# flynn-nrg/izpi

Measured on AMD Instinct MI355X. Metric: Msamples/sec (pixels x spp) at 1024x1024/512spp, higher is better.
Workload: dtype f64

## Files before the change

### izpi_amd/csrc/izpi_dev.h

```cpp
#pragma once
#include <hip/hip_runtime.h>
#include <stdint.h>
#include "../../include/izpi_gpu.h"
#include "gomath.h"

#define IZPI_DEV __device__ __forceinline__

namespace izd {

__host__ __device__ inline bool ref_is_leaf(int32_t r) { return r <= -2; }
__host__ __device__ inline int32_t leaf_start(int32_t r) { return (-r - 1) >> 3; }
__host__ __device__ inline int32_t leaf_count(int32_t r) { return (-r - 1) & 7; }
__host__ __device__ inline int32_t make_leaf_ref(int32_t start, int32_t count) { return -(1 + ((start << 3) | count)); }

struct alignas(16) GInner {
  float mnx[4], mny[4], mnz[4], mxx[4], mxy[4], mxz[4];
  int32_t child[4];
  int32_t pad[4];
};
struct alignas(64) GInnerQ {
  float org[3];
  uint32_t ex;
  uint32_t q[6];
  int32_t child[4];
  uint32_t pad[2];
};
static_assert(sizeof(GInnerQ) == 64, "GInnerQ is 64 B");
__host__ __device__ inline float qdecode(float org, uint32_t q, float s) {
  const float p = (float)q * s;
  return org + p;
}
struct alignas(16) GLeaf {
  float mn[3], mx[3];
  int32_t start, count;
};
struct alignas(16) GPrim {
  double a[9];
  uint32_t kind;
  uint32_t index;
};
struct alignas(32) GShade {
  double n[3];
  uint32_t ref;
  uint32_t mk;
};
__host__ __device__ inline uint32_t gs_mat(const GShade& g) { return g.mk >> 8; }
__host__ __device__ inline uint32_t gs_kind(const GShade& g) { return (g.mk >> 2) & 63u; }
__host__ __device__ inline uint32_t gs_cflags(const GShade& g) { return g.mk & 3u; }
struct alignas(16) GTriTex {
  double uv[6];
  double tg[3], bt[3];
};
struct alignas(16) GTriVerts {
  double v1[3], v2[3];
};
struct alignas(16) GLight {
  double v0[3], v1[3], v2[3], e1[3], e2[3], n[3];
  double area;
  double c0[3], c1[3], radius, t0, t1;
  double cz[3];
  uint32_t kind, index;
};

enum { TEXF_RGBA = 0, TEXF_GRAY = 1, TEXF_OTHER = 2, TEXF_NONE = 3 };
struct alignas(16) TexSlot {
  uint64_t off;
  uint32_t w, hf;
};
struct alignas(64) MatTex {
  TexSlot s[4];
};

struct DevScene {
  const GInner* inner;
  const GInnerQ* innerq;
  const GLeaf* leaves;
  const GPrim* prims;
  const GShade* shade;
  const GTriTex* tritex;
  const GLight* lights;
  const izpi_material* materials;
  const izpi_texture* textures;
  const double4* mat_const;
  const MatTex* mat_tex;
  const double* texels;
  const double* spd_wl;
  const double* spd_val;
  int32_t root;
  uint32_t num_lights;
  uint32_t nan_free_bounds;
  uint32_t leaf_shortcut;
  uint32_t tri_only;
  uint32_t no_pathlen;
  uint32_t num_inner;
  uint32_t num_prims;
  izpi_camera cam;
  uint32_t lds_bytes;
  uint32_t time_free;
  uint32_t quantized;
#ifdef IZPI_SHADOW
  const GInner* sh_inner;
  const GLeaf* sh_leaves;
  const GPrim* sh_prims;
#endif
};

struct RenderParams {
  uint32_t width, height, spp, max_depth;
  uint32_t chunk_spp;
  uint32_t s0;
  uint32_t num_pixels;
  uint32_t tile_w, tile_h;
  uint32_t total_units;
  uint32_t lanes;
  uint32_t num_bg_spd;
  const uint32_t* tiles;
  const double* bg_wl;
  const double* bg_val;
  double background[3];
  uint64_t seed;
  double* out;
  double* recs;
  uint32_t* head;
  unsigned long long* counters;
  uint32_t* error;
};

struct Lcg {
  uint32_t s;
  IZPI_DEV double next() {
    s = 1664525u * s + 1013904223u;
    return (double)s / 4294967296.0;
  }
};
IZPI_DEV uint64_t splitmix64(uint64_t x) {
  uint64_t z = x + 0x9E3779B97F4A7C15ull;
  z = (z ^ (z >> 30)) * 0xBF58476D1CE4E5B9ull;
  z = (z ^ (z >> 27)) * 0x94D049BB133111EBull;
  return z ^ (z >> 31);
}
#define IZPI_CAMERA_STREAM_SALT 0xD6E8FEB86659FD93ull

IZPI_DEV int64_t go_int(double x) {
  if (x != x || x >= 9223372036854775808.0 || x < -9223372036854775808.0) return INT64_MIN;
  return (int64_t)x;
}

struct V3 { double x, y, z; };
IZPI_DEV V3 mk(double x, double y, double z) { V3 r; r.x = x; r.y = y; r.z = z; return r; }
IZPI_DEV V3 ld3(const double* p) { return mk(p[0], p[1], p[2]); }
IZPI_DEV V3 add(V3 a, V3 b) { return mk(a.x + b.x, a.y + b.y, a.z + b.z); }
IZPI_DEV V3 sub(V3 a, V3 b) { return mk(a.x - b.x, a.y - b.y, a.z - b.z); }
IZPI_DEV V3 mul(V3 a, V3 b) { return mk(a.x * b.x, a.y * b.y, a.z * b.z); }
IZPI_DEV V3 smul(V3 a, double t) { return mk(a.x * t, a.y * t, a.z * t); }
IZPI_DEV bool sdiv_plain(double x) {
  return ((uint32_t)(__double2hiint(x) >> 20) & 0x7FFu) - (1023u - 300u) <= 600u;
}
IZPI_DEV V3 sdiv(V3 a, double t) {
  const int px = (int)sdiv_plain(a.x) | (int)(a.x == 0.0), py = (int)sdiv_plain(a.y) | (int)(a.y == 0.0),
            pz = (int)sdiv_plain(a.z) | (int)(a.z == 0.0);
  const bool plain = ((int)sdiv_plain(t) & px & py & pz) != 0;
  if (plain) {
    double r = __builtin_amdgcn_rcp(t);
    double e = __builtin_fma(-t, r, 1.0);
    r = __builtin_fma(r, e, r);
    e = __builtin_fma(-t, r, 1.0);
    r = __builtin_fma(r, e, r);
    auto q1 = [&](double n) {
      const double q = n * r;
      const double res = __builtin_fma(-t, q, n);
      return __builtin_amdgcn_div_fixup(__builtin_amdgcn_div_fmas(res, r, q, false), t, n);
    };
    return mk(q1(a.x), q1(a.y), q1(a.z));
  }
  return mk(a.x / t, a.y / t, a.z / t);
}
IZPI_DEV double dot(V3 a, V3 b) { return (a.x * b.x) + (a.y * b.y) + (a.z * b.z); }
IZPI_DEV V3 cross(V3 a, V3 b) { return mk((a.y * b.z) - (a.z * b.y), -((a.x * b.z) - (a.z * b.x)), (a.x * b.y) - (a.y * b.x)); }
IZPI_DEV double sqlen(V3 a) { return (a.x * a.x) + (a.y * a.y) + (a.z * a.z); }
IZPI_DEV double length(V3 a) { return gm::sqrt(sqlen(a)); }
IZPI_DEV V3 unit(V3 a) { return sdiv(a, length(a)); }
IZPI_DEV V3 lerp(V3 a, V3 b, double t) {
  return mk((1 - t) * a.x + t * b.x, (1 - t) * a.y + t * b.y, (1 - t) * a.z + t * b.z);
}
IZPI_DEV bool bad(double x) { return x != x || gm::is_inf(x, 0); }
IZPI_DEV V3 denan(V3 v) { return mk(bad(v.x) ? 0.0 : v.x, bad(v.y) ? 0.0 : v.y, bad(v.z) ? 0.0 : v.z); }

struct Onb {
  V3 u, v, w;
  IZPI_DEV void build(V3 n) {
    w = unit(n);
    V3 a = gm::abs(w.x) > 0.9 ? mk(0, 1, 0) : mk(1, 0, 0);
    v = unit(cross(w, a));
    u = cross(w, v);
  }
  IZPI_DEV V3 local(V3 a) const { return add(add(smul(u, a.x), smul(v, a.y)), smul(w, a.z)); }
};

IZPI_DEV V3 random_cosine_direction(Lcg& r) {
  double r1 = r.next();
  double r2 = r.next();
  double z = gm::sqrt(1 - r2);
  double phi = 6.283185307179586 * r1;
  double sp, cp;
  gm::sincos_nonneg(phi, &sp, &cp);
  double x = cp * 2 * gm::sqrt(r2);
  double y = sp * 2 * gm::sqrt(r2);
  return mk(x, y, z);
}
IZPI_DEV V3 random_to_sphere(double radius, double dist2, Lcg& r) {
  double r1 = r.next();
  double r2 = r.next();
  double z = 1 + r2 * (gm::sqrt(1 - radius * radius / dist2) - 1);
  double phi = 6.283185307179586 * r1;
  double sp, cp;
  gm::sincos_nonneg(phi, &sp, &cp);
  double x = cp * gm::sqrt(1 - z * z);
  double y = sp * gm::sqrt(1 - z * z);
  return mk(x, y, z);
}
IZPI_DEV V3 random_in_unit_sphere(Lcg& r) {
  for (;;) {
    double x = r.next(), y = r.next(), z = r.next();
    V3 p = sub(smul(mk(x, y, z), 2.0), mk(1.0, 1.0, 1.0));
    if (sqlen(p) < 1.0) return p;
  }
}

IZPI_DEV float max32(float a, float b) { return a > b ? a : b; }
IZPI_DEV float min32(float a, float b) { return a < b ? a : b; }
IZPI_DEV bool slab(float mnx, float mny, float mnz, float mxx, float mxy, float mxz, float ox, float oy, float oz,
                   float ix, float iy, float iz, float tmax) {
  float t0x = (mnx - ox) * ix, t1x = (mxx - ox) * ix;
  if (t0x > t1x) { float t = t0x; t0x = t1x; t1x = t; }
  float t0y = (mny - oy) * iy, t1y = (mxy - oy) * iy;
  if (t0y > t1y) { float t = t0y; t0y = t1y; t1y = t; }
  float t0z = (mnz - oz) * iz, t1z = (mxz - oz) * iz;
  if (t0z > t1z) { float t = t0z; t0z = t1z; t1z = t; }
  float tn = max32(max32(t0x, t0y), t0z);
  float tf = min32(min32(t1x, t1y), t1z);
  return tn <= tf && tf >= 0 && tn <= tmax;
}

typedef float f32x2 __attribute__((ext_vector_type(2)));
IZPI_DEV uint32_t slab4_fast(float4 mnx, float4 mny, float4 mnz, float4 mxx, float4 mxy, float4 mxz, float ox, float oy,
                             float oz, float ix, float iy, float iz, float tmax) {
  const f32x2 o_x = {ox, ox}, o_y = {oy, oy}, o_z = {oz, oz};
  const f32x2 i_x = {ix, ix}, i_y = {iy, iy}, i_z = {iz, iz};
  const f32x2 a0x = (f32x2{mnx.x, mnx.y} - o_x) * i_x, a1x = (f32x2{mnx.z, mnx.w} - o_x) * i_x;
  const f32x2 b0x = (f32x2{mxx.x, mxx.y} - o_x) * i_x, b1x = (f32x2{mxx.z, mxx.w} - o_x) * i_x;
  const f32x2 a0y = (f32x2{mny.x, mny.y} - o_y) * i_y, a1y = (f32x2{mny.z, mny.w} - o_y) * i_y;
  const f32x2 b0y = (f32x2{mxy.x, mxy.y} - o_y) * i_y, b1y = (f32x2{mxy.z, mxy.w} - o_y) * i_y;
  const f32x2 a0z = (f32x2{mnz.x, mnz.y} - o_z) * i_z, a1z = (f32x2{mnz.z, mnz.w} - o_z) * i_z;
  const f32x2 b0z = (f32x2{mxz.x, mxz.y} - o_z) * i_z, b1z = (f32x2{mxz.z, mxz.w} - o_z) * i_z;
  const float t0x[4] = {a0x.x, a0x.y, a1x.x, a1x.y}, t1x[4] = {b0x.x, b0x.y, b1x.x, b1x.y};
  const float t0y[4] = {a0y.x, a0y.y, a1y.x, a1y.y}, t1y[4] = {b0y.x, b0y.y, b1y.x, b1y.y};
  const float t0z[4] = {a0z.x, a0z.y, a1z.x, a1z.y}, t1z[4] = {b0z.x, b0z.y, b1z.x, b1z.y};
  uint32_t m = 0;
#pragma unroll
  for (int i = 0; i < 4; i++) {
    const float tn = __builtin_fmaxf(__builtin_fmaxf(__builtin_fminf(t0x[i], t1x[i]), __builtin_fminf(t0y[i], t1y[i])),
                                     __builtin_fminf(t0z[i], t1z[i]));
    const float tf = __builtin_fminf(__builtin_fminf(__builtin_fmaxf(t0x[i], t1x[i]), __builtin_fmaxf(t0y[i], t1y[i])),
                                     __builtin_fmaxf(t0z[i], t1z[i]));
    m |= (tn <= tf && tf >= 0.0f && tn <= tmax) ? (1u << i) : 0u;
  }
  return m;
}
IZPI_DEV bool ray_fast_ok(float ox, float oy, float oz, float ix, float iy, float iz) {
  const float inf = __builtin_huge_valf();
  return __builtin_fabsf(ox) < inf && __builtin_fabsf(oy) < inf && __builtin_fabsf(oz) < inf &&
         __builtin_fabsf(ix) < inf && __builtin_fabsf(iy) < inf && __builtin_fabsf(iz) < inf &&
         ix != 0.0f && iy != 0.0f && iz != 0.0f;
}

IZPI_DEV bool tri_intersect(const double* a, V3 o, V3 d, double tmin, double tmax, double& t, double& u, double& v) {
  const double eps = 1e-8;
  V3 v0 = mk(a[0], a[1], a[2]), e1 = mk(a[3], a[4], a[5]), e2 = mk(a[6], a[7], a[8]);
  V3 h = cross(d, e2);
  double aa = dot(e1, h);
  if (gm::abs(aa) < eps) return false;
  double f = 1.0 / aa;
  V3 s = sub(o, v0);
  u = f * dot(s, h);
  if (u < -eps || u > 1.0 + eps) return false;
  V3 q = cross(s, e1);
  v = f * dot(d, q);
  if (v < -eps || u + v > 1.0 + eps) return false;
  t = f * dot(e2, q);
  if (t < tmin || t > tmax) return false;
  return true;
}
IZPI_DEV bool tri_intersect_no_tmax(const double* a, V3 o, V3 d, double tmin, double& t, double& u, double& v) {
  const double eps = 1e-8;
  V3 v0 = mk(a[0], a[1], a[2]), e1 = mk(a[3], a[4], a[5]), e2 = mk(a[6], a[7], a[8]);
  V3 h = cross(d, e2);
  double aa = dot(e1, h);
  if (gm::abs(aa) < eps) return false;
  double f = 1.0 / aa;
  V3 s = sub(o, v0);
  u = f * dot(s, h);
  if (u < -eps || u > 1.0 + eps) return false;
  V3 q = cross(s, e1);
  v = f * dot(d, q);
  if (v < -eps || u + v > 1.0 + eps) return false;
  t = f * dot(e2, q);
  if (t < tmin) return false;
  return true;
}
IZPI_DEV V3 sph_center(const double* a, double time) {
  V3 c0 = mk(a[0], a[1], a[2]), c1 = mk(a[3], a[4], a[5]);
  return add(c0, smul(sub(c1, c0), ((time - a[7]) / (a[8] - a[7]))));
}
IZPI_DEV bool sph_intersect_at(V3 center, double radius, V3 o, V3 d, double tmin, double tmax, double& t, int& root) {
  V3 oc = sub(o, center);
  double aa = dot(d, d);
  double b = dot(oc, d);
  double c = dot(oc, oc) - (radius * radius);
  double disc = (b * b) - (aa * c);
  if (disc > 0) {
    double temp = (-b - gm::sqrt(b * b - aa * c)) / aa;
    if (temp < tmax && temp > tmin) { t = temp; root = 0; return true; }
    temp = (-b + gm::sqrt(b * b - aa * c)) / aa;
    if (temp < tmax && temp > tmin) { t = temp; root = 1; return true; }
  }
  return false;
}
IZPI_DEV bool sph_roots(V3 center, double radius, V3 o, V3 d, double& t0, double& t1) {
  V3 oc = sub(o, center);
  double aa = dot(d, d);
  double b = dot(oc, d);
  double c = dot(oc, oc) - (radius * radius);
  double disc = (b * b) - (aa * c);
  if (!(disc > 0)) return false;
  t0 = (-b - gm::sqrt(b * b - aa * c)) / aa;
  t1 = (-b + gm::sqrt(b * b - aa * c)) / aa;
  return true;
}
IZPI_DEV bool sph_intersect(const double* a, V3 o, V3 d, double time, double tmin, double tmax, double& t, int& root) {
  return sph_intersect_at(sph_center(a, time), a[6], o, d, tmin, tmax, t, root);
}

}
```

### izpi_amd/csrc/trace.hip

```cpp
#include "izpi_kern.h"

constexpr uint32_t BVH_LDS_BYTES = 4096;
template <int S, int WPE, bool DIST, bool TRI, bool LB, bool RL, bool Q>
__global__ void __launch_bounds__(256) __attribute__((amdgpu_waves_per_eu(WPE))) k_trace2(const DevScene sc, const WaveParams wp, unsigned long long* counters,
                                                uint32_t* err, int32_t* spill, uint32_t spill_stride, uint32_t prim_w,
                                                uint32_t tchunk, uint32_t refill_min) {
  static_assert((S & (S - 1)) == 0, "ring size must be a power of two");
  static_assert(!LB || DIST, "the LDS-resident BVH instance runs the distributed leaf tests");
  static_assert(!RL || (DIST && (TRI || LB)), "the LDS-resident ray instances: triangle-only global BVH, or the BVH in LDS");
  static_assert(!Q || !LB, "the quantised nodes are read from global memory");
  constexpr bool UVL = !RL, UVS = RL && LB, DUV = !RL || LB;
  typedef float v4f __attribute__((ext_vector_type(4)));
  typedef double v2d __attribute__((ext_vector_type(2)));
  typedef const __attribute__((address_space(3))) v4f LF4;
  typedef const __attribute__((address_space(3))) v2d LD2;
  __shared__ float4 bvh_lds[LB ? BVH_LDS_BYTES / 16 : 1];
  LF4* const l_inner = (LF4*)bvh_lds;
  LF4* const l_leaves = l_inner + (size_t)8 * (LB ? sc.num_inner : 0);
  LD2* const l_prims = (LD2*)(l_leaves + (size_t)2 * (LB ? sc.num_prims : 0));
  if constexpr (LB) {
    const uint32_t ni = 8 * sc.num_inner, nl = 2 * sc.num_prims, np5 = 5 * sc.num_prims;
    for (uint32_t t = threadIdx.x; t < ni + nl + np5; t += 256)
      bvh_lds[t] = t < ni ? reinterpret_cast<const float4*>(sc.inner)[t]
                          : (t < ni + nl ? reinterpret_cast<const float4*>(sc.leaves)[t - ni]
                                         : reinterpret_cast<const float4*>(sc.prims)[t - ni - nl]);
    __syncthreads();
  }
  __shared__ int32_t lds_stack[S * 256];
  __shared__ uint32_t dist_owner[DIST ? 260 : 1];
  __shared__ double dist_t[DIST ? 260 : 1], dist_u[DIST && DUV ? 260 : 1], dist_v[DIST && DUV ? 260 : 1];
  __shared__ double2 lds_uv[UVL ? 256 : 1];
  __shared__ double2 ray_lds[RL ? 3 * 256 : 1];
  const uint32_t wbase = threadIdx.x & ~63u;
  int32_t* stk = lds_stack + threadIdx.x;
  int32_t* gsp = spill + blockIdx.x * 256 + threadIdx.x;
  const uint32_t lane = threadIdx.x & 63;
  const uint32_t n = *wp.in_count;
  if (wp.pool_ctr && blockIdx.x == 0) pool_publish(wp.pool_ctr);
  if (wp.out_count && blockIdx.x == 0 && threadIdx.x == 0) *wp.out_count = 0;
  if (wp.out_park && blockIdx.x == 0 && threadIdx.x == 0) *wp.out_park = 0;
  const bool read_kind = wp.read_kind != 0 || (wp.in_park && *wp.in_park != 0);
  const uint32_t nwaves = gridDim.x * 4u;
  const uint32_t chunk = min(tchunk, max(16u, (n + nwaves - 1u) / nwaves));
  const uint32_t first = chunk;
  if ((uint64_t)(blockIdx.x * 4u + (threadIdx.x >> 6)) * first >= n) return;
  uint64_t c_rays = 0, c_nodes = 0, c_tri = 0, c_sph = 0;
  uint64_t c_nstep = 0, c_pstep = 0, c_short = 0;
  bool busy = false, in_prim = false;
  bool exhausted = false;
  uint32_t qi = 0;
  uint32_t lkind = RAY_MAIN;
  double tmax = 0;
  float ix = 0, iy = 0, iz = 0, ox = 0, oy = 0, oz = 0;
  int32_t cur = -1, pk = 0, pend = 0;
  int sp = 0, low = 0;
  int clean_from = 0;
  int32_t bprim = -1;
  bool fast = false;
#ifdef IZPI_SHADOW
  uint64_t c_spill_st = 0, c_spill_ld = 0;
  uint32_t sh_acc = 0;
#endif
  uint32_t c_pos = __builtin_amdgcn_readfirstlane((blockIdx.x * 4u + (threadIdx.x >> 6)) * first);
  uint32_t c_end = c_pos + first < n ? c_pos + first : n;
#ifdef IZPI_TRACE_CLOCKS
  uint64_t k_refill = 0, k_node = 0, k_prim = 0, k_adv = 0, k0 = 0, k1 = 0;
#define IZPI_CLK(v) (v) = __builtin_readcyclecounter()
#else
#define IZPI_CLK(v) (void)0
#endif
  for (;;) {
    IZPI_CLK(k0);
    const uint64_t idle = __ballot(!busy);
    if (idle != 0) {
      const uint32_t nidle = (uint32_t)__popcll(idle);
      if (!exhausted && (nidle >= refill_min || idle == ~0ull) && c_pos >= c_end) {
        uint32_t b = 0;
        if (lane == 0) b = atomicAdd(wp.trace_next, chunk);
        b = __builtin_amdgcn_readfirstlane(b) + nwaves * first;
        if (b >= n) exhausted = true;
        c_pos = b;
        c_end = b + chunk < n ? b + chunk : n;
      }
      if (!exhausted && (nidle >= refill_min || idle == ~0ull) && c_pos < c_end) {
        const uint32_t take = nidle < c_end - c_pos ? nidle : c_end - c_pos;
        const uint32_t base = c_pos;
        c_pos += take;
        bool main_ray = false;
        const uint32_t rank = (uint32_t)__popcll(idle & ((1ull << lane) - 1));
        const uint32_t my = base + rank;
        if (!busy && rank < take) {
          const uint32_t k = read_kind ? sld(wp.in.kind + my) : (uint32_t)RAY_MAIN;
          RayOD r;
          if constexpr (RL) {
            r = sld(wp.in.ray + my);
            const double2* rp = reinterpret_cast<const double2*>(&r);
            const double2 r0 = rp[0], r1 = rp[1], r2 = rp[2];
            ray_lds[3 * threadIdx.x] = r0; ray_lds[3 * threadIdx.x + 1] = r1; ray_lds[3 * threadIdx.x + 2] = r2;
          } else {
            r = wp.in.ray[my];
          }
          if (!(k & (RAY_PARKED | RAY_DEAD)) && (uint64_t)__double_as_longlong(r.o[0]) != DEAD_BITS) {
            qi = my;
            lkind = k;
            tmax = ray_tmax(wp.in, my, k);
            main_ray = kind_of(k) == RAY_MAIN;
            ix = (float)(1.0 / r.d[0]); iy = (float)(1.0 / r.d[1]); iz = (float)(1.0 / r.d[2]);
            ox = (float)r.o[0]; oy = (float)r.o[1]; oz = (float)r.o[2];
            fast = sc.nan_free_bounds && ray_fast_ok(ox, oy, oz, ix, iy, iz);
            cur = sc.root;
            sp = 0; low = 0; clean_from = 0;
            in_prim = false;
            bprim = -1;
            busy = cur != -1;
            if (!busy) {
              if ((UVL || UVS) && wp.hit_uv) {
                double2* rec = wp.in.hit + ((size_t)my << 1);
                sst(rec, hit_pack(0.0, -1)); sst(rec + 1, make_double2(0.0, 0.0));
              } else {
                sst(wp.in.hit + my, hit_pack(0.0, -1));
              }
            }
          }
        }
        c_rays += (uint64_t)__popcll(__ballot(main_ray));
        __builtin_amdgcn_s_waitcnt(0x0F70);
      } else if (exhausted && idle == ~0ull) {
        break;
      }
    }
    const uint64_t m_prim = __ballot(busy && in_prim);
    const uint64_t m_node = __ballot(busy && !in_prim);
    if ((m_prim | m_node) == 0) continue;
    const uint32_t n_prim = (uint32_t)__popcll(m_prim), n_node = (uint32_t)__popcll(m_node);
    bool advance = false;
    bool leaf_next = false;
    int32_t next = -1;
#ifdef IZPI_TRACE_CLOCKS
    IZPI_CLK(k1); k_refill += k1 - k0; k0 = k1;
    const bool clk_prim = n_prim * prim_w >= n_node * 16u;
#endif
    if (n_prim * prim_w >= n_node * 16u) {
      if constexpr (DIST) {
        const uint32_t cnt = (busy && in_prim) ? (uint32_t)(pend - pk) : 0u;
        const uint64_t lt = (1ull << lane) - 1;
        const uint32_t base = (uint32_t)__popcll(__ballot(cnt & 1u) & lt) + 2u * (uint32_t)__popcll(__ballot(cnt & 2u) & lt) +
                              4u * (uint32_t)__popcll(__ballot(cnt & 4u) & lt);
        const bool served = cnt > 0 && base + cnt <= 64;
        const uint64_t ms = __ballot(served);
        const int last = 63 - __clzll((long long)ms);
        const uint32_t total = (uint32_t)__shfl((int)(base + cnt), last);
        {
          const uint32_t e = ((uint32_t)pk << 6) | lane;
          uint32_t* dq = dist_owner + wbase + base;
          if (served) dq[0] = e;
          if (served && cnt > 1) dq[1] = e + 64u;
          if (served && cnt > 2) dq[2] = e + 128u;
          if (served && cnt > 3) dq[3] = e + 192u;
        }
        __builtin_amdgcn_wave_barrier();
        const uint32_t ent = lane < total ? dist_owner[wbase + lane] : lane;
        const uint32_t ow = ent & 63u;
        const uint32_t oqi = (uint32_t)__shfl((int)qi, (int)ow);
        const uint32_t okind = (uint32_t)__shfl((int)lkind, (int)ow);
        if (lane < total) {
          const int32_t pi = (int32_t)(ent >> 6);
          double2 r0, r1, r2;
          if constexpr (RL) {
            const uint32_t ro = 3 * (wbase + ow);
            r0 = ray_lds[ro]; r1 = ray_lds[ro + 1]; r2 = ray_lds[ro + 2];
          } else {
            const double2* rp = reinterpret_cast<const double2*>(wp.in.ray + oqi);
            r0 = rp[0]; r1 = rp[1]; r2 = rp[2];
          }
          const double otmin = ray_tmin(wp.in, oqi, okind);
          double2 p0, p1, p2, p3, p4;
          if constexpr (LB) {
            LD2* pp = l_prims + (size_t)5 * pi;
            const v2d a0 = pp[0], a1 = pp[1], a2 = pp[2], a3 = pp[3], a4 = pp[4];
            p0 = make_double2(a0.x, a0.y); p1 = make_double2(a1.x, a1.y); p2 = make_double2(a2.x, a2.y);
            p3 = make_double2(a3.x, a3.y); p4 = make_double2(a4.x, a4.y);
          } else {
            const double2* pp = reinterpret_cast<const double2*>(sc.prims + pi);
            p0 = pp[0]; p1 = pp[1]; p2 = pp[2]; p3 = pp[3]; p4 = pp[4];
#ifdef IZPI_SHADOW
            if (IZPI_SHADOW & 4) {
              const uint4* sq = reinterpret_cast<const uint4*>(sc.sh_prims + pi);
              const uint4 s0 = sq[0], s1 = sq[1], s2 = sq[2], s3 = sq[3], s4 = sq[4];
              sh_acc ^= s0.x ^ s1.y ^ s2.z ^ s3.w ^ s4.x;
            }
#endif
          }
          const double pa[9] = {p0.x, p0.y, p1.x, p1.y, p2.x, p2.y, p3.x, p3.y, p4.x};
          double t = 0, u = 0, v = 0;
          const V3 o = mk(r0.x, r0.y, r1.x), d = mk(r1.y, r2.x, r2.y);
          uint32_t flags;
          if (TRI || (uint32_t)__double2loint(p4.y) == IZPI_PRIM_TRIANGLE) {
            flags = tri_intersect_no_tmax(pa, o, d, otmin, t, u, v) ? 1u : 0u;
          } else {
            const double time = (RL && LB) || sc.time_free ? pa[7] : (wp.in.time ? wp.in.time[oqi] : 0.0);
            flags = 2u;
            if (sph_roots(sph_center(pa, time), pa[6], o, d, t, u))
              flags |= 1u | (t > otmin ? 4u : 0u) | (u > otmin ? 8u : 0u);
          }
          dist_t[wbase + lane] = t;
          if constexpr (DUV) { dist_u[wbase + lane] = u; dist_v[wbase + lane] = v; }
          dist_owner[wbase + lane] = flags;
        }
        const uint32_t n_sph_tests = TRI ? 0u : (uint32_t)__popcll(__ballot(lane < total && (dist_owner[wbase + lane] & 2u)));
        __builtin_amdgcn_wave_barrier();
        if (served && (TRI || n_sph_tests == 0)) {
          const uint32_t j0 = wbase + base;
          uint32_t f[4];
          double tt[4];
#pragma unroll
          for (uint32_t i = 0; i < 4; i++) { f[i] = dist_owner[j0 + i]; tt[i] = dist_t[j0 + i]; }
          int32_t acc = -1;
#pragma unroll
          for (uint32_t i = 0; i < 4; i++)
            if (i < cnt && (f[i] & 1u) && !(tt[i] > tmax)) { tmax = tt[i]; acc = (int32_t)i; }
          if (acc >= 0) {
            if constexpr (UVL) lds_uv[threadIdx.x] = make_double2(dist_u[j0 + acc], dist_v[j0 + acc]);
            if constexpr (UVS)
              if (wp.hit_uv) sst(wp.in.hit + ((size_t)qi << 1) + 1, make_double2(dist_u[j0 + acc], dist_v[j0 + acc]));
            bprim = pk + acc;
            clean_from = sp;
          }
          pk = pend;
          in_prim = false;
          advance = true;
        } else if (!TRI && served) {
          int32_t acc = -1;
          double acc_u = 0, acc_v = 0;
          for (uint32_t i = 0; i < cnt; i++) {
            const uint32_t j = wbase + base + i;
            const uint32_t f = dist_owner[j];
            if (!(f & 1u)) continue;
            if (!(f & 2u)) {
              const double t = dist_t[j];
              if (!(t > tmax)) { tmax = t; acc = (int32_t)j; acc_u = dist_u[j]; acc_v = dist_v[j]; bprim = pk + (int32_t)i; }
            } else {
              const double ta = dist_t[j], tb = dist_u[j];
              if (ta < tmax && (f & 4u)) { tmax = ta; acc = (int32_t)j; acc_u = 0.0; acc_v = 0.0; bprim = pk + (int32_t)i; }
              else if (tb < tmax && (f & 8u)) { tmax = tb; acc = (int32_t)j; acc_u = 1.0; acc_v = 0.0; bprim = pk + (int32_t)i; }
            }
          }
          if (acc >= 0) {
            if constexpr (UVS) {
              if (wp.hit_uv) sst(wp.in.hit + ((size_t)qi << 1) + 1, make_double2(acc_u, acc_v));
            } else {
              lds_uv[threadIdx.x] = make_double2(acc_u, acc_v);
            }
            clean_from = sp;
          }
          pk = pend;
          in_prim = false;
          advance = true;
        }
        __builtin_amdgcn_wave_barrier();
        c_tri += total - n_sph_tests;
        c_sph += n_sph_tests;
        c_pstep++;
      } else {
      bool is_tri = false;
      if (busy && in_prim) {
        const double2* rp = reinterpret_cast<const double2*>(wp.in.ray + qi);
        const double2 r0 = rp[0], r1 = rp[1], r2 = rp[2];
        const V3 o = mk(r0.x, r0.y, r1.x), d = mk(r1.y, r2.x, r2.y);
        const double tmin = ray_tmin(wp.in, qi, lkind);
        const double2* pp = reinterpret_cast<const double2*>(sc.prims + pk);
        const double2 p0 = pp[0], p1 = pp[1], p2 = pp[2], p3 = pp[3], p4 = pp[4];
        const double pa[9] = {p0.x, p0.y, p1.x, p1.y, p2.x, p2.y, p3.x, p3.y, p4.x};
        is_tri = TRI || (uint32_t)__double2loint(p4.y) == IZPI_PRIM_TRIANGLE;
        if (is_tri) {
          double t, u, v;
          if (tri_intersect(pa, o, d, tmin, tmax, t, u, v)) {
            tmax = t; bprim = pk; lds_uv[threadIdx.x] = make_double2(u, v); clean_from = sp;
          }
        } else if (!TRI) {
          const double time = wp.in.time ? wp.in.time[qi] : 0.0;
          double t; int root;
          if (sph_intersect(pa, o, d, time, tmin, tmax, t, root)) {
            tmax = t; bprim = pk; lds_uv[threadIdx.x] = make_double2((double)root, 0.0); clean_from = sp;
          }
        }
        pk++;
        if (pk == pend) { in_prim = false; advance = true; }
      }
      const uint32_t n_tri = (uint32_t)__popcll(__ballot(is_tri));
      c_tri += n_tri;
      c_sph += n_prim - n_tri;
      c_pstep++;
      }
    } else {
      c_nodes += n_node;
      c_nstep++;
      const bool wave_fast = __ballot(busy && !in_prim && !fast) == 0;
      if (__ballot(busy && !in_prim && sp + 3 - low > S) != 0) {
        if (busy && !in_prim) {
          while (sp + 3 - low > S) {
            gsp[(size_t)low * spill_stride] = stk[(low & (S - 1)) * 256];
            low++;
#ifdef IZPI_SHADOW
            c_spill_st++;
#endif
          }
        }
      }
      if (busy && !in_prim) {
        const float tm = (float)tmax;
        const bool is_leaf = ref_is_leaf(cur);
        float4 q0, q1, mnz_, mxx_, mxy_, mxz_;
        int4 ch_;
        if constexpr (LB) {
          LF4* lp = is_leaf ? l_leaves + (size_t)2 * leaf_start(cur) : l_inner + (size_t)8 * cur;
          LF4* np = is_leaf ? l_inner : lp;
          const v4f a0 = lp[0], a1 = lp[1], a2 = np[2], a3 = np[3], a4 = np[4], a5 = np[5], c = np[6];
          q0 = make_float4(a0.x, a0.y, a0.z, a0.w); q1 = make_float4(a1.x, a1.y, a1.z, a1.w);
          mnz_ = make_float4(a2.x, a2.y, a2.z, a2.w); mxx_ = make_float4(a3.x, a3.y, a3.z, a3.w);
          mxy_ = make_float4(a4.x, a4.y, a4.z, a4.w); mxz_ = make_float4(a5.x, a5.y, a5.z, a5.w);
          ch_ = make_int4(__float_as_int(c.x), __float_as_int(c.y), __float_as_int(c.z), __float_as_int(c.w));
        } else if constexpr (Q) {
          const float4* lp = reinterpret_cast<const float4*>(is_leaf ? (const void*)(sc.leaves + leaf_start(cur))
                                                                     : (const void*)(sc.innerq + cur));
          const float4* np = is_leaf ? reinterpret_cast<const float4*>(sc.innerq) : lp;
          q0 = lp[0]; q1 = lp[1];
          const float4 c2 = np[2], c3 = np[3];
          const uint32_t ex = __float_as_uint(q0.w);
          const float sx = __uint_as_float((ex & 0xFFu) << 23), sy = __uint_as_float(((ex >> 8) & 0xFFu) << 23),
                      sz = __uint_as_float(((ex >> 16) & 0xFFu) << 23);
          auto dec4 = [](float w, float o, float sc_) {
            const uint32_t b = __float_as_uint(w);
            return make_float4(__builtin_fmaf((float)(b & 0xFFu), sc_, o), __builtin_fmaf((float)((b >> 8) & 0xFFu), sc_, o),
                               __builtin_fmaf((float)((b >> 16) & 0xFFu), sc_, o), __builtin_fmaf((float)(b >> 24), sc_, o));
          };
          const float4 dmnx = dec4(q1.x, q0.x, sx), dmny = dec4(q1.y, q0.y, sy), dmnz = dec4(q1.z, q0.z, sz);
          const float4 dmxx = dec4(q1.w, q0.x, sx), dmxy = dec4(c2.x, q0.y, sy), dmxz = dec4(c2.y, q0.z, sz);
          const float4 l0 = q0, l1 = q1;
          q0 = is_leaf ? l0 : dmnx;
          q1 = is_leaf ? l1 : make_float4(dmny.x, dmny.y, dmny.z, dmny.w);
          mnz_ = dmnz; mxx_ = dmxx; mxy_ = dmxy; mxz_ = dmxz;
          ch_ = make_int4(__float_as_int(c2.z), __float_as_int(c2.w), __float_as_int(c3.x), __float_as_int(c3.y));
        } else {
          const float4* lp = reinterpret_cast<const float4*>(is_leaf ? (const void*)(sc.leaves + leaf_start(cur))
                                                                     : (const void*)(sc.inner + cur));
          const float4* np = is_leaf ? reinterpret_cast<const float4*>(sc.inner) : lp;
          q0 = lp[0]; q1 = lp[1];
          mnz_ = np[2]; mxx_ = np[3]; mxy_ = np[4]; mxz_ = np[5];
          ch_ = *reinterpret_cast<const int4*>(np + 6);
#ifdef IZPI_SHADOW
          if ((IZPI_SHADOW & 1) && !is_leaf) {
            const uint4* sq = reinterpret_cast<const uint4*>(sc.sh_inner + cur);
            const uint4 s0 = sq[0], s1 = sq[1], s2 = sq[2], s3 = sq[3], s4 = sq[4], s5 = sq[5], s6 = sq[6];
            sh_acc ^= s0.x ^ s1.y ^ s2.z ^ s3.w ^ s4.x ^ s5.y ^ s6.z;
          }
          if ((IZPI_SHADOW & 2) && is_leaf) {
            const uint4* sq = reinterpret_cast<const uint4*>(sc.sh_leaves + leaf_start(cur));
            const uint4 s0 = sq[0], s1 = sq[1];
            sh_acc ^= s0.x ^ s1.y;
          }
#endif
        }
        const float4 mnx = q0;
        const float4 mny = make_float4(is_leaf ? q0.y : q1.x, q1.y, q1.z, q1.w);
        const float4 mnz = make_float4(is_leaf ? q0.z : mnz_.x, mnz_.y, mnz_.z, mnz_.w);
        const float4 mxx = make_float4(is_leaf ? q0.w : mxx_.x, mxx_.y, mxx_.z, mxx_.w);
        const float4 mxy = make_float4(is_leaf ? q1.x : mxy_.x, mxy_.y, mxy_.z, mxy_.w);
        const float4 mxz = make_float4(is_leaf ? q1.y : mxz_.x, mxz_.y, mxz_.z, mxz_.w);
        const int4 ch = make_int4(is_leaf ? cur : ch_.x, ch_.y, ch_.z, ch_.w);
        uint32_t hm;
        if (wave_fast) {
          hm = slab4_fast(mnx, mny, mnz, mxx, mxy, mxz, ox, oy, oz, ix, iy, iz, tm);
        } else {
          const float amnx[4] = {mnx.x, mnx.y, mnx.z, mnx.w}, amny[4] = {mny.x, mny.y, mny.z, mny.w},
                      amnz[4] = {mnz.x, mnz.y, mnz.z, mnz.w}, amxx[4] = {mxx.x, mxx.y, mxx.z, mxx.w},
                      amxy[4] = {mxy.x, mxy.y, mxy.z, mxy.w}, amxz[4] = {mxz.x, mxz.y, mxz.z, mxz.w};
          hm = 0;
#pragma unroll
          for (int i = 0; i < 4; i++)
            if (slab(amnx[i], amny[i], amnz[i], amxx[i], amxy[i], amxz[i], ox, oy, oz, ix, iy, iz, tm)) hm |= 1u << i;
        }
        const uint32_t valid = is_leaf ? 1u
                                       : ((ch.x != -1 ? 1u : 0u) | (ch.y != -1 ? 2u : 0u) | (ch.z != -1 ? 4u : 0u) |
                                          (ch.w != -1 ? 8u : 0u));
        const uint32_t m = hm & valid;
        const int32_t c01 = (m & 1u) ? ch.x : ch.y, c23 = (m & 4u) ? ch.z : ch.w;
        next = m == 0 ? -1 : ((m & 3u) ? c01 : c23);
        const bool enter = ref_is_leaf(next) && (is_leaf || sc.leaf_shortcut);
        leaf_next = enter && !is_leaf;
        in_prim = enter;
        pk = enter ? leaf_start(next) : pk;
        pend = enter ? leaf_start(next) + leaf_count(next) : pend;
        next = enter ? -1 : next;
        const uint32_t rest = m & (m - 1u);
        const int np_ = __builtin_popcount(rest);
        const int32_t e0 = (rest & 2u) ? ch.y : ((rest & 4u) ? ch.z : ch.w);
        const int32_t e1 = ((rest & 6u) == 6u) ? ch.z : ch.w;
        stk[(sp & (S - 1)) * 256] = e0;
        stk[((sp + 1) & (S - 1)) * 256] = e1;
        stk[((sp + 2) & (S - 1)) * 256] = ch.w;
        if (sp + np_ > 64) atomicOr(err, 1u);
        sp += np_;
        advance = !enter;
      }
    }
#ifdef IZPI_TRACE_CLOCKS
    IZPI_CLK(k1); if (clk_prim) k_prim += k1 - k0; else k_node += k1 - k0; k0 = k1;
#endif
    {
      const bool do_pop = advance && next == -1 && sp > 0;
      const bool do_fin = advance && next == -1 && sp == 0;
      const int spn = sp - 1;
      int32_t top = *(volatile __attribute__((address_space(3))) int32_t*)&lds_stack[threadIdx.x + (spn & (S - 1)) * 256];
      if (__ballot(do_pop && spn < low) != 0) {
        if (do_pop && spn < low) {
          top = gsp[(size_t)spn * spill_stride];
          low = spn;
#ifdef IZPI_SHADOW
          c_spill_ld++;
#endif
        }
        __builtin_amdgcn_s_waitcnt(0x0F70);
      }
      cur = (advance && next != -1) ? next : (do_pop ? top : cur);
      sp = do_pop ? spn : sp;
      const bool lf = do_pop && ref_is_leaf(top) && spn >= clean_from && sc.leaf_shortcut;
      in_prim = in_prim || lf;
      leaf_next = leaf_next || lf;
      pk = lf ? leaf_start(top) : pk;
      pend = lf ? leaf_start(top) + leaf_count(top) : pend;
      clean_from = (do_pop && spn < clean_from) ? spn : clean_from;
      if (do_fin) {
        const double2 uv = (UVL && bprim >= 0) ? lds_uv[threadIdx.x] : make_double2(0.0, 0.0);
        if ((UVL || UVS) && wp.hit_uv) {
          double2* rec = wp.in.hit + ((size_t)qi << 1);
          sst(rec, hit_pack(bprim >= 0 ? tmax : 0.0, bprim));
          if (!UVS || bprim < 0) sst(rec + 1, uv);
        } else {
          sst(wp.in.hit + qi, hit_pack(bprim >= 0 ? tmax : 0.0, bprim));
        }
        busy = false;
      }
    }
    const uint64_t n_short = (uint64_t)__popcll(__ballot(leaf_next));
    c_nodes += n_short;
    c_short += n_short;
#ifdef IZPI_TRACE_CLOCKS
    IZPI_CLK(k1); k_adv += k1 - k0;
#endif
  }
#ifdef IZPI_TRACE_CLOCKS
  if (lane == 0) {
    atomicAdd(counters + CNT_CLK_REFILL, (unsigned long long)k_refill);
    atomicAdd(counters + CNT_CLK_NODE, (unsigned long long)k_node);
    atomicAdd(counters + CNT_CLK_PRIM, (unsigned long long)k_prim);
    atomicAdd(counters + CNT_CLK_ADV, (unsigned long long)k_adv);
  }
#endif
#ifdef IZPI_SHADOW
  {
    if (c_spill_st) atomicAdd(counters + CNT_CLK_REFILL, (unsigned long long)c_spill_st);
    if (c_spill_ld) atomicAdd(counters + CNT_CLK_NODE, (unsigned long long)c_spill_ld);
    if (sh_acc == 0x9E3779B9u) atomicOr(err, 0u);
  }
#endif
  if (lane == 0) {
    count_add(wp.cpart, counters, CNT_RAYS, c_rays);
    count_add(wp.cpart, counters, CNT_NODES, c_nodes);
    count_add(wp.cpart, counters, CNT_TRI, c_tri);
    count_add(wp.cpart, counters, CNT_SPH, c_sph);
    count_add(wp.cpart, counters, CNT_NSTEP, c_nstep);
    count_add(wp.cpart, counters, CNT_PSTEP, c_pstep);
    count_add(wp.cpart, counters, CNT_SHORT, c_short);
  }
}


#define IZPI_T2_LIST(X)                                                                                           \
  X(true, false, false, false, false) X(true, true, false, false, false) X(false, false, false, false, false)        \
  X(false, true, false, false, false) X(true, false, true, false, false) X(true, true, true, false, false)           \
  X(true, true, false, true, false) X(true, false, true, true, false) X(true, true, true, true, false)               \
  X(true, false, false, false, true) X(true, true, false, false, true) X(true, true, false, true, true)
constexpr int ring_of(bool lb, bool rl) { return lb && rl ? 8 : TRACE_RING; }

int make_tracer(izpi_ctx* ctx, const izpi_render_tuning& tu, bool need_uv, Tracer* t) {
  *t = Tracer();
  if (tu.flags & IZPI_TUNE_NO_DIST) t->p2 = false;
  if (ctx->num_prims >= (1u << 26)) t->p2 = false;
  t->tri = ctx->sc.tri_only != 0 && !(tu.flags & IZPI_TUNE_GENERAL_TRACE);
  t->lds_bvh = t->p2 && !(tu.flags & IZPI_TUNE_NO_LDS_BVH) &&
               (uint64_t)ctx->sc.num_inner * sizeof(GInner) + (uint64_t)ctx->sc.num_prims * (sizeof(GLeaf) + sizeof(GPrim)) <= BVH_LDS_BYTES;
  if (t->lds_bvh) {
    t->refill_min = 40;
    t->prim_w = 24;
  }
  t->ray_lds = t->p2 && ((t->tri && !t->lds_bvh && !need_uv) || (t->lds_bvh && (t->tri || ctx->sc.time_free))) &&
               !(tu.flags & IZPI_TUNE_NO_RAY_LDS);
  t->qnodes = ctx->sc.quantized && t->p2 && !t->lds_bvh && !(tu.flags & IZPI_TUNE_NO_QNODES);
  if (tu.prim_weight) t->prim_w = tu.prim_weight;
  if (tu.trace_chunk) t->tchunk = tu.trace_chunk;
  if (tu.refill_min) t->refill_min = std::min<uint32_t>(64, tu.refill_min);
  int rc = IZPI_ERR_INVALID;
  ctx->err = "no k_trace2 instance for this scene and tuning";
#define IZPI_T2_OCC(P, T, L, R, Q)                                                               \
  if (t->p2 == P && t->tri == T && t->lds_bvh == L && t->ray_lds == R && t->qnodes == Q) \
    rc = resident_blocks(ctx, k_trace2<ring_of(L, R), TRACE_WPE, P, T, L, R, Q>, &t->blocks);
  IZPI_T2_LIST(IZPI_T2_OCC)
#undef IZPI_T2_OCC
  if (rc) return rc;
  t->spill_bytes = (size_t)t->blocks * 256 * 64 * sizeof(int32_t);
  return IZPI_OK;
}

void launch_trace(izpi_ctx* ctx, const DevScene& sc, const Tracer& t, const WaveParams& wp, hipStream_t st, int32_t* spill) {
  const dim3 g(t.blocks), b(256);
  const uint32_t stride = (uint32_t)t.blocks * 256;
#define IZPI_T2_LAUNCH(P, T, L, R, Q)                                                                          \
  if (t.p2 == P && t.tri == T && t.lds_bvh == L && t.ray_lds == R && t.qnodes == Q) {                          \
    hipLaunchKernelGGL((k_trace2<ring_of(L, R), TRACE_WPE, P, T, L, R, Q>), g, b, 0, st, sc, wp, ctx->d_counters, \
                       misc(ctx, 1), spill, stride, t.prim_w, t.tchunk, t.refill_min);                        \
    return;                                                                                                    \
  }
  IZPI_T2_LIST(IZPI_T2_LAUNCH)
#undef IZPI_T2_LAUNCH
}
```

Before: 2418.

## Move traversal control masks to wave-uniform scalar ballots and branchless tests

Reworks the BVH traversal loop so per-lane state checks are kept in 64-bit wave-level ballot masks. Idle, primitive and node lanes are derived from sp<0 and pk<pend, the child-hit selection and stack pushes are computed from scalar masks with inverse-ballot, and the rank and base counts use mbcnt. The per-wave slow-ray mask is cached at refill, and the spill reload check is skipped until a spill has happened. The triangle test without tmax becomes branchless. The aim is to cut VALU compare/select and per-lane bitmask work and move it to the SALU. The cost is more ballot instructions and a subtle change to the sp/busy state encoding, which risks correctness bugs.

```diff
diff --git a/izpi_amd/csrc/izpi_dev.h b/izpi_amd/csrc/izpi_dev.h
--- a/izpi_amd/csrc/izpi_dev.h
+++ b/izpi_amd/csrc/izpi_dev.h
@@ -243,8 +243,8 @@
 }
 
 typedef float f32x2 __attribute__((ext_vector_type(2)));
-IZPI_DEV uint32_t slab4_fast(float4 mnx, float4 mny, float4 mnz, float4 mxx, float4 mxy, float4 mxz, float ox, float oy,
-                             float oz, float ix, float iy, float iz, float tmax) {
+IZPI_DEV void slab4_fast(float4 mnx, float4 mny, float4 mnz, float4 mxx, float4 mxy, float4 mxz, float ox, float oy,
+                         float oz, float ix, float iy, float iz, float tmax, uint64_t (&h)[4]) {
   const f32x2 o_x = {ox, ox}, o_y = {oy, oy}, o_z = {oz, oz};
   const f32x2 i_x = {ix, ix}, i_y = {iy, iy}, i_z = {iz, iz};
   const f32x2 a0x = (f32x2{mnx.x, mnx.y} - o_x) * i_x, a1x = (f32x2{mnx.z, mnx.w} - o_x) * i_x;
@@ -256,16 +256,14 @@
   const float t0x[4] = {a0x.x, a0x.y, a1x.x, a1x.y}, t1x[4] = {b0x.x, b0x.y, b1x.x, b1x.y};
   const float t0y[4] = {a0y.x, a0y.y, a1y.x, a1y.y}, t1y[4] = {b0y.x, b0y.y, b1y.x, b1y.y};
   const float t0z[4] = {a0z.x, a0z.y, a1z.x, a1z.y}, t1z[4] = {b0z.x, b0z.y, b1z.x, b1z.y};
-  uint32_t m = 0;
 #pragma unroll
   for (int i = 0; i < 4; i++) {
     const float tn = __builtin_fmaxf(__builtin_fmaxf(__builtin_fminf(t0x[i], t1x[i]), __builtin_fminf(t0y[i], t1y[i])),
                                      __builtin_fminf(t0z[i], t1z[i]));
     const float tf = __builtin_fminf(__builtin_fminf(__builtin_fmaxf(t0x[i], t1x[i]), __builtin_fmaxf(t0y[i], t1y[i])),
                                      __builtin_fmaxf(t0z[i], t1z[i]));
-    m |= (tn <= tf && tf >= 0.0f && tn <= tmax) ? (1u << i) : 0u;
-  }
-  return m;
+    h[i] = __builtin_amdgcn_ballot_w64(tn <= tf) & __builtin_amdgcn_ballot_w64(tf >= 0.0f) & __builtin_amdgcn_ballot_w64(tn <= tmax);
+  }
 }
 IZPI_DEV bool ray_fast_ok(float ox, float oy, float oz, float ix, float iy, float iz) {
   const float inf = __builtin_huge_valf();
@@ -296,17 +294,14 @@
   V3 v0 = mk(a[0], a[1], a[2]), e1 = mk(a[3], a[4], a[5]), e2 = mk(a[6], a[7], a[8]);
   V3 h = cross(d, e2);
   double aa = dot(e1, h);
-  if (gm::abs(aa) < eps) return false;
   double f = 1.0 / aa;
   V3 s = sub(o, v0);
   u = f * dot(s, h);
-  if (u < -eps || u > 1.0 + eps) return false;
   V3 q = cross(s, e1);
   v = f * dot(d, q);
-  if (v < -eps || u + v > 1.0 + eps) return false;
   t = f * dot(e2, q);
-  if (t < tmin) return false;
-  return true;
+  const bool r0 = gm::abs(aa) < eps, r1 = (u < -eps) | (u > 1.0 + eps), r2 = (v < -eps) | (u + v > 1.0 + eps), r3 = t < tmin;
+  return !(r0 | r1 | r2 | r3);
 }
 IZPI_DEV V3 sph_center(const double* a, double time) {
   V3 c0 = mk(a[0], a[1], a[2]), c1 = mk(a[3], a[4], a[5]);
diff --git a/izpi_amd/csrc/trace.hip b/izpi_amd/csrc/trace.hip
--- a/izpi_amd/csrc/trace.hip
+++ b/izpi_amd/csrc/trace.hip
@@ -1,6 +1,10 @@
 #include "izpi_kern.h"
 
 constexpr uint32_t BVH_LDS_BYTES = 4096;
+__device__ __forceinline__ bool lane_of(uint64_t mask) { return __builtin_amdgcn_inverse_ballot_w64(mask); }
+__device__ __forceinline__ uint32_t lanes_below(uint64_t mask) {
+  return __builtin_amdgcn_mbcnt_hi((uint32_t)(mask >> 32), __builtin_amdgcn_mbcnt_lo((uint32_t)mask, 0u));
+}
 template <int S, int WPE, bool DIST, bool TRI, bool LB, bool RL, bool Q>
 __global__ void __launch_bounds__(256) __attribute__((amdgpu_waves_per_eu(WPE))) k_trace2(const DevScene sc, const WaveParams wp, unsigned long long* counters,
                                                 uint32_t* err, int32_t* spill, uint32_t spill_stride, uint32_t prim_w,
@@ -53,10 +57,12 @@
   double tmax = 0;
   float ix = 0, iy = 0, iz = 0, ox = 0, oy = 0, oz = 0;
   int32_t cur = -1, pk = 0, pend = 0;
-  int sp = 0, low = 0;
+  int sp = -1, low = 0;
   int clean_from = 0;
   int32_t bprim = -1;
   bool fast = false;
+  uint64_t m_slow = ~0ull;
+  bool any_spill = false;
 #ifdef IZPI_SHADOW
   uint64_t c_spill_st = 0, c_spill_ld = 0;
   uint32_t sh_acc = 0;
@@ -69,12 +75,20 @@
 #else
 #define IZPI_CLK(v) (void)0
 #endif
+#ifdef IZPI_STEP_MARKS
+#define IZPI_MARK(name) asm volatile("; IZPI_MARK " name)
+#else
+#define IZPI_MARK(name) (void)0
+#endif
   for (;;) {
     IZPI_CLK(k0);
-    const uint64_t idle = __ballot(!busy);
+    IZPI_MARK("head");
+    const uint64_t idle = __builtin_amdgcn_ballot_w64(sp < 0);
+    uint64_t idle_now = idle;
     if (idle != 0) {
       const uint32_t nidle = (uint32_t)__popcll(idle);
       if (!exhausted && (nidle >= refill_min || idle == ~0ull) && c_pos >= c_end) {
+        IZPI_MARK("dequeue");
         uint32_t b = 0;
         if (lane == 0) b = atomicAdd(wp.trace_next, chunk);
         b = __builtin_amdgcn_readfirstlane(b) + nwaves * first;
@@ -83,11 +97,12 @@
         c_end = b + chunk < n ? b + chunk : n;
       }
       if (!exhausted && (nidle >= refill_min || idle == ~0ull) && c_pos < c_end) {
+        IZPI_MARK("refill");
         const uint32_t take = nidle < c_end - c_pos ? nidle : c_end - c_pos;
         const uint32_t base = c_pos;
         c_pos += take;
         bool main_ray = false;
-        const uint32_t rank = (uint32_t)__popcll(idle & ((1ull << lane) - 1));
+        const uint32_t rank = lanes_below(idle);
         const uint32_t my = base + rank;
         if (!busy && rank < take) {
           const uint32_t k = read_kind ? sld(wp.in.kind + my) : (uint32_t)RAY_MAIN;
@@ -109,10 +124,10 @@
             ox = (float)r.o[0]; oy = (float)r.o[1]; oz = (float)r.o[2];
             fast = sc.nan_free_bounds && ray_fast_ok(ox, oy, oz, ix, iy, iz);
             cur = sc.root;
-            sp = 0; low = 0; clean_from = 0;
+            busy = cur != -1;
+            sp = busy ? 0 : -1; low = 0; clean_from = 0;
             in_prim = false;
             bprim = -1;
-            busy = cur != -1;
             if (!busy) {
               if ((UVL || UVS) && wp.hit_uv) {
                 double2* rec = wp.in.hit + ((size_t)my << 1);
@@ -124,13 +139,16 @@
           }
         }
         c_rays += (uint64_t)__popcll(__ballot(main_ray));
+        m_slow = __ballot(!fast);
+        idle_now = __builtin_amdgcn_ballot_w64(sp < 0);
         __builtin_amdgcn_s_waitcnt(0x0F70);
       } else if (exhausted && idle == ~0ull) {
         break;
       }
     }
-    const uint64_t m_prim = __ballot(busy && in_prim);
-    const uint64_t m_node = __ballot(busy && !in_prim);
+    IZPI_MARK("pick");
+    const uint64_t m_prim = __builtin_amdgcn_ballot_w64(pk < pend);
+    const uint64_t m_node = ~(m_prim | idle_now);
     if ((m_prim | m_node) == 0) continue;
     const uint32_t n_prim = (uint32_t)__popcll(m_prim), n_node = (uint32_t)__popcll(m_node);
     bool advance = false;
@@ -142,14 +160,14 @@
 #endif
     if (n_prim * prim_w >= n_node * 16u) {
       if constexpr (DIST) {
-        const uint32_t cnt = (busy && in_prim) ? (uint32_t)(pend - pk) : 0u;
-        const uint64_t lt = (1ull << lane) - 1;
-        const uint32_t base = (uint32_t)__popcll(__ballot(cnt & 1u) & lt) + 2u * (uint32_t)__popcll(__ballot(cnt & 2u) & lt) +
-                              4u * (uint32_t)__popcll(__ballot(cnt & 4u) & lt);
-        const bool served = cnt > 0 && base + cnt <= 64;
-        const uint64_t ms = __ballot(served);
+        IZPI_MARK("prim");
+        const uint32_t cnt = (uint32_t)(pend - pk);
+        const uint32_t base = lanes_below(__ballot(cnt & 1u)) + 2u * lanes_below(__ballot(cnt & 2u)) +
+                              4u * lanes_below(__ballot(cnt & 4u));
+        const uint64_t ms = m_prim & __builtin_amdgcn_ballot_w64(base + cnt <= 64);
+        const bool served = lane_of(ms);
         const int last = 63 - __clzll((long long)ms);
-        const uint32_t total = (uint32_t)__shfl((int)(base + cnt), last);
+        const uint32_t total = (uint32_t)__builtin_amdgcn_readlane((int)(base + cnt), last);
         {
           const uint32_t e = ((uint32_t)pk << 6) | lane;
           uint32_t* dq = dist_owner + wbase + base;
@@ -293,10 +311,12 @@
       c_pstep++;
       }
     } else {
+      IZPI_MARK("node");
       c_nodes += n_node;
       c_nstep++;
-      const bool wave_fast = __ballot(busy && !in_prim && !fast) == 0;
-      if (__ballot(busy && !in_prim && sp + 3 - low > S) != 0) {
+      const bool wave_fast = (m_node & m_slow) == 0;
+      if ((m_node & __builtin_amdgcn_ballot_w64(sp + 3 - low > S)) != 0) {
+        any_spill = true;
         if (busy && !in_prim) {
           while (sp + 3 - low > S) {
             gsp[(size_t)low * spill_stride] = stk[(low & (S - 1)) * 256];
@@ -368,34 +388,37 @@
         const float4 mxy = make_float4(is_leaf ? q1.x : mxy_.x, mxy_.y, mxy_.z, mxy_.w);
         const float4 mxz = make_float4(is_leaf ? q1.y : mxz_.x, mxz_.y, mxz_.z, mxz_.w);
         const int4 ch = make_int4(is_leaf ? cur : ch_.x, ch_.y, ch_.z, ch_.w);
-        uint32_t hm;
+        uint64_t hit[4];
         if (wave_fast) {
-          hm = slab4_fast(mnx, mny, mnz, mxx, mxy, mxz, ox, oy, oz, ix, iy, iz, tm);
+          slab4_fast(mnx, mny, mnz, mxx, mxy, mxz, ox, oy, oz, ix, iy, iz, tm, hit);
         } else {
           const float amnx[4] = {mnx.x, mnx.y, mnx.z, mnx.w}, amny[4] = {mny.x, mny.y, mny.z, mny.w},
                       amnz[4] = {mnz.x, mnz.y, mnz.z, mnz.w}, amxx[4] = {mxx.x, mxx.y, mxx.z, mxx.w},
                       amxy[4] = {mxy.x, mxy.y, mxy.z, mxy.w}, amxz[4] = {mxz.x, mxz.y, mxz.z, mxz.w};
-          hm = 0;
 #pragma unroll
           for (int i = 0; i < 4; i++)
-            if (slab(amnx[i], amny[i], amnz[i], amxx[i], amxy[i], amxz[i], ox, oy, oz, ix, iy, iz, tm)) hm |= 1u << i;
-        }
-        const uint32_t valid = is_leaf ? 1u
-                                       : ((ch.x != -1 ? 1u : 0u) | (ch.y != -1 ? 2u : 0u) | (ch.z != -1 ? 4u : 0u) |
-                                          (ch.w != -1 ? 8u : 0u));
-        const uint32_t m = hm & valid;
-        const int32_t c01 = (m & 1u) ? ch.x : ch.y, c23 = (m & 4u) ? ch.z : ch.w;
-        next = m == 0 ? -1 : ((m & 3u) ? c01 : c23);
+            hit[i] = __builtin_amdgcn_ballot_w64(slab(amnx[i], amny[i], amnz[i], amxx[i], amxy[i], amxz[i], ox, oy, oz, ix, iy, iz, tm));
+        }
+        const uint64_t m_inner = __builtin_amdgcn_ballot_w64(cur >= -1);
+        const uint64_t b0 = hit[0] & __builtin_amdgcn_ballot_w64(ch.x != -1),
+                       b1 = hit[1] & m_inner & __builtin_amdgcn_ballot_w64(ch.y != -1),
+                       b2 = hit[2] & m_inner & __builtin_amdgcn_ballot_w64(ch.z != -1),
+                       b3 = hit[3] & m_inner & __builtin_amdgcn_ballot_w64(ch.w != -1);
+        next = lane_of(b3) ? ch.w : -1;
+        next = lane_of(b2) ? ch.z : next;
+        next = lane_of(b1) ? ch.y : next;
+        next = lane_of(b0) ? ch.x : next;
         const bool enter = ref_is_leaf(next) && (is_leaf || sc.leaf_shortcut);
         leaf_next = enter && !is_leaf;
         in_prim = enter;
         pk = enter ? leaf_start(next) : pk;
         pend = enter ? leaf_start(next) + leaf_count(next) : pend;
         next = enter ? -1 : next;
-        const uint32_t rest = m & (m - 1u);
-        const int np_ = __builtin_popcount(rest);
-        const int32_t e0 = (rest & 2u) ? ch.y : ((rest & 4u) ? ch.z : ch.w);
-        const int32_t e1 = ((rest & 6u) == 6u) ? ch.z : ch.w;
+        const uint64_t r1 = b0 & b1, r2 = (b0 | b1) & b2, r3 = (b0 | b1 | b2) & b3;
+        const int np_ = (int)lane_of(r1) + (int)lane_of(r2) + (int)lane_of(r3);
+        const int32_t e0z = lane_of(r2) ? ch.z : ch.w;
+        const int32_t e0 = lane_of(r1) ? ch.y : e0z;
+        const int32_t e1 = lane_of(r1 & r2) ? ch.z : ch.w;
         stk[(sp & (S - 1)) * 256] = e0;
         stk[((sp + 1) & (S - 1)) * 256] = e1;
         stk[((sp + 2) & (S - 1)) * 256] = ch.w;
@@ -408,11 +431,12 @@
     IZPI_CLK(k1); if (clk_prim) k_prim += k1 - k0; else k_node += k1 - k0; k0 = k1;
 #endif
     {
+      IZPI_MARK("advance");
       const bool do_pop = advance && next == -1 && sp > 0;
       const bool do_fin = advance && next == -1 && sp == 0;
       const int spn = sp - 1;
       int32_t top = *(volatile __attribute__((address_space(3))) int32_t*)&lds_stack[threadIdx.x + (spn & (S - 1)) * 256];
-      if (__ballot(do_pop && spn < low) != 0) {
+      if (any_spill && __ballot(do_pop && spn < low) != 0) {
         if (do_pop && spn < low) {
           top = gsp[(size_t)spn * spill_stride];
           low = spn;
@@ -423,7 +447,7 @@
         __builtin_amdgcn_s_waitcnt(0x0F70);
       }
       cur = (advance && next != -1) ? next : (do_pop ? top : cur);
-      sp = do_pop ? spn : sp;
+      sp = (advance && next == -1) ? spn : sp;
       const bool lf = do_pop && ref_is_leaf(top) && spn >= clean_from && sc.leaf_shortcut;
       in_prim = in_prim || lf;
       leaf_next = leaf_next || lf;
```

New measurement: 2553, median of 6. +5.5%, better.
